# noah-aviel-dove/signals

Measured on AMD Instinct MI355X. Metric: rendered Msamples/s (48 kHz, 256-sample blocks), higher is better.
Workload: dtype f64; 1 GPU; C2: 1024-voice Fixed->Sine->LowPass->Gain->SumBus(stereo) per GPU, 48 kHz, 256-frame blocks, 4096 blocks per batch (f32 storage, f64 phase/recurrence); engine schedule = fused voice chain + bus: sig_fused_voice_bus (Sine->LowPass->Gain->SumBus in ONE launch, its voice tiles added in fixed order by the same kernel; no per-voice sample touches HBM); voices_per_gpu=1024, block_frames=256, start_position=0, parallelism=voices sharded 1024/GPU x1; single process, no collective, rccl_ranks=0

## Files before the change

### signals_amd/csrc/fused_voice.hip

```cpp
#include <cstdlib>

#include "sig_fused_launch.h"

sig_fused::Tuning& sig_fused::tuning() {
    static Tuning t = [] {
        auto env = [](const char* name, int dflt) { const char* e = getenv(name); return e ? atoi(e) : dflt; };
        Tuning u;
        u.vpt = env("SIG_FUSED_VPT", 0); u.span = env("SIG_FUSED_SPAN", 0);
        u.steady = env("SIG_FUSED_STEADY", -1); u.scan = env("SIG_FUSED_SCAN", -1);
        if (u.steady == 2) { u.steady = 1; u.tile_sum_kernel = 1; }
        if (u.steady == 3) { u.steady = 1; u.mix_f32 = 1; }
        return u;
    }();
    return t;
}

namespace {

enum Sink { SINK_VOICES, SINK_MIX, SINK_BUS };
struct FusedCall {
    int osc_kind, filt_type; int32_t rate; int64_t position;
    int32_t block_frames, nblocks, context, voices;
    const double* hertz; int32_t hertz_stride; const double* phase; int32_t phase_stride;
    const double* cutoff; int32_t cutoff_stride; const double* gain; int32_t gain_stride;
    float* out; int64_t out_ld; int32_t* status; void* stream;
    Sink sink = SINK_VOICES;
    bool rows = false;
    int32_t cutoff_rows = 1, gain_rows = 1;
    int pair_op = 0, kind2 = 0;
    const double* hertz2 = nullptr; int32_t hertz2_stride = 0; const double* phase2 = nullptr; int32_t phase2_stride = 0;
    const double* mix = nullptr; int32_t mix_stride = 0;
    int32_t hertz_rows = 1, phase_rows = 1; const double* hertz_hist = nullptr; const double* phase_hist = nullptr;
    bool devpos = false; const int64_t* position_dev = nullptr;
    const float* matrix = nullptr;
    const double* bus_gains = nullptr; int64_t bus_gains_ld = 0; int32_t bus_channels = 0; double* workspace = nullptr;
    double* consts = nullptr; int32_t consts_ready = 0; int force_walk = 0;
};

bool stride_ok(int32_t s) { return (s | 1) == 1; }

bool call_ok(const FusedCall& c)
{
    const bool bus = c.sink == SINK_BUS;
    if (c.filt_type != SIG_FILT_LOWPASS && c.filt_type != SIG_FILT_HIGHPASS) return false;
    if (!(c.rate > 0 && (c.devpos ? c.position_dev != nullptr : c.position >= 0))) return false;
    if (!(c.block_frames >= 0 && c.nblocks >= 0 && c.context >= 0 && c.voices >= 0)) return false;
    if (!(c.hertz && c.cutoff && c.out && c.out_ld >= (bus ? c.bus_channels : c.voices))) return false;
    if (!(stride_ok(c.hertz_stride) && stride_ok(c.phase_stride) && stride_ok(c.cutoff_stride) && stride_ok(c.gain_stride))) return false;
    if (!((c.cutoff_rows == 1 || c.cutoff_rows == c.nblocks) && (c.gain_rows == 1 || c.gain_rows == c.nblocks))) return false;
    if (c.pair_op != 0 && !((c.pair_op == 1 || c.pair_op == 2) && c.kind2 >= SIG_OSC_SINE && c.kind2 <= SIG_OSC_TRIANGLE && c.hertz2 &&
                            stride_ok(c.hertz2_stride) && stride_ok(c.phase2_stride) && stride_ok(c.mix_stride) && (c.pair_op == 2 || c.mix)))
        return false;
    if ((c.hertz_hist || c.phase_hist) && c.block_frames < c.context) return false;
    if (!((c.hertz_rows == 1 || (c.hertz_rows == c.nblocks && c.hertz_hist)) &&
          (c.phase_rows == 1 || (c.phase_rows == c.nblocks && c.phase_hist)) && (!c.phase_hist || c.phase))) return false;
    if (c.sink == SINK_MIX && !(c.matrix && c.voices % 64 == 0)) return false;
    if (bus && !(c.workspace && (c.bus_gains ? c.bus_gains_ld >= c.voices : c.bus_channels == 1))) return false;
    return true;
}

int run_call(const FusedCall& c)
{
    SIG_CHECK_ARG(call_ok(c));
    if (c.block_frames == 0 || c.nblocks == 0 || c.voices == 0) return 0;
    const bool bus = c.sink == SINK_BUS;
    FusedArgs a{c.filt_type, (double)c.rate, c.devpos ? 0 : c.position, c.block_frames, c.nblocks, c.context, c.voices,
                c.hertz, c.hertz_stride, c.phase, c.phase_stride, c.cutoff, c.cutoff_stride, c.gain, c.gain_stride,
                bus ? nullptr : c.out, bus ? 0 : c.out_ld, 0, c.status, c.devpos ? c.position_dev : nullptr};
    a.mix = c.matrix;
    a.consts_ext = c.consts; a.consts_ready = c.consts_ready; a.force_walk = c.force_walk;
    a.cutoff_rows = c.cutoff_rows; a.gain_rows = c.gain_rows;
    a.hertz_rows = c.hertz_rows; a.phase_rows = c.phase_rows; a.hertz_hist = c.hertz_hist; a.phase_hist = c.phase_hist;
    a.pair_op = c.pair_op; a.kind2 = c.kind2; a.hertz2 = c.hertz2; a.hs2 = c.hertz2_stride; a.phase2 = c.phase2; a.ps2 = c.phase2_stride;
    a.mixrow = c.mix; a.ms = c.mix_stride;
    const BusArgs busargs = bus ? BusArgs{c.bus_gains, c.bus_gains_ld, c.workspace, (int64_t)c.block_frames * c.nblocks}
                                : BusArgs{nullptr, 0, nullptr, 0};
    hipStream_t s = static_cast<hipStream_t>(c.stream);
    if (c.rows) {
        SIG_CHECK_ARG(!bus || c.bus_channels == 1 || c.bus_channels == 2);
        return dispatch_rows(bus ? c.bus_channels : 0, c.osc_kind, a, busargs, c.out, c.out_ld, s);
    }
    switch (c.sink) {
        case SINK_BUS: return dispatch_bus(c.gain != nullptr, c.osc_kind, c.bus_channels, a, busargs, c.out, c.out_ld, s);
        case SINK_MIX: return dispatch_mix(c.gain != nullptr, c.osc_kind, a, s);
        default: return dispatch_chain(c.gain != nullptr, c.osc_kind, a, s);
    }
}

void set_rows(FusedCall& c, int32_t cutoff_rows, int32_t gain_rows) { c.rows = true; c.cutoff_rows = cutoff_rows; c.gain_rows = gain_rows; }

void set_bus(FusedCall& c, const double* bus_gains, int64_t bus_gains_ld, int32_t bus_channels, double* workspace)
{
    c.sink = SINK_BUS; c.bus_gains = bus_gains; c.bus_gains_ld = bus_gains_ld; c.bus_channels = bus_channels; c.workspace = workspace;
}
// ... 107 lines not shown
                                      int32_t block_frames, int32_t nblocks, int32_t context, int32_t voices,
                                      const double* hertz, int32_t hertz_stride, int32_t hertz_rows, const double* hertz_hist,
                                      const double* phase, int32_t phase_stride, int32_t phase_rows, const double* phase_hist,
                                      const double* cutoff, int32_t cutoff_stride, int32_t cutoff_rows,
                                      const double* gain, int32_t gain_stride, int32_t gain_rows,
                                      const double* bus_gains, int64_t bus_gains_ld, int32_t bus_channels,
                                      double* workspace, float* out, int64_t out_ld, int32_t* status, void* stream)
{
    FusedCall c{osc_kind, filt_type, rate, position, block_frames, nblocks, context, voices, hertz, hertz_stride, phase, phase_stride,
                cutoff, cutoff_stride, gain, gain_stride, out, out_ld, status, stream};
    set_rows(c, cutoff_rows, gain_rows);
    set_fm(c, hertz_rows, hertz_hist, phase_rows, phase_hist);
    set_bus(c, bus_gains, bus_gains_ld, bus_channels, workspace);
    return run_call(c);
}

extern "C" int sig_fused_osc_biquad_devpos(int osc_kind, int filt_type, int32_t rate, const int64_t* position_dev,
                                           int32_t block_frames, int32_t nblocks, int32_t context, int32_t voices,
                                           const double* hertz, int32_t hertz_stride, const double* phase, int32_t phase_stride,
                                           const double* cutoff, int32_t cutoff_stride,
                                           const double* gain, int32_t gain_stride,
                                           float* out, int64_t out_ld, int32_t* status, void* stream)
{
    FusedCall c{osc_kind, filt_type, rate, 0, block_frames, nblocks, context, voices, hertz, hertz_stride, phase, phase_stride,
                cutoff, cutoff_stride, gain, gain_stride, out, out_ld, status, stream};
    c.devpos = true; c.position_dev = position_dev;
    return run_call(c);
}

namespace {
__global__ void advance_kernel(int64_t* p, int64_t delta) { *p += delta; }
}

extern "C" int sig_advance_position(int64_t* position_dev, int64_t delta, void* stream)
{
    SIG_CHECK_ARG(position_dev != nullptr);
    advance_kernel<<<1, 1, 0, static_cast<hipStream_t>(stream)>>>(position_dev, delta);
    return sig_launch_status();
}

extern "C" int sig_fused_osc_biquad_mix(int osc_kind, int filt_type, int32_t rate, int64_t position,
                                        int32_t block_frames, int32_t nblocks, int32_t context, int32_t voices,
                                        const double* hertz, int32_t hertz_stride, const double* phase, int32_t phase_stride,
                                        const double* cutoff, int32_t cutoff_stride,
                                        const double* gain, int32_t gain_stride,
                                        const float* matrix, float* out, int64_t out_ld, int32_t* status, void* stream)
{
    FusedCall c{osc_kind, filt_type, rate, position, block_frames, nblocks, context, voices, hertz, hertz_stride, phase, phase_stride,
                cutoff, cutoff_stride, gain, gain_stride, out, out_ld, status, stream};
    c.sink = SINK_MIX; c.matrix = matrix;
    return run_call(c);
}

extern "C" int sig_fused_geometry(int32_t voices, int32_t block_frames, int32_t nblocks, int32_t context,
                                  int32_t* voices_per_lane, int32_t* blocks_per_lane)
{
    SIG_CHECK_ARG(voices >= 0 && block_frames >= 0 && nblocks >= 0 && context >= 0 && voices_per_lane && blocks_per_lane);
    FusedArgs a{};
    a.N = block_frames; a.K = nblocks; a.ctx = context; a.voices = voices;
    int vpt = 1, span = 1;
    pick_geometry(a, 4, vpt, span);
    *voices_per_lane = vpt;
    *blocks_per_lane = span;
    return 0;
}

extern "C" int sig_fused_voice_bus_plan(int osc_kind, int64_t position, int32_t voices, int32_t block_frames, int32_t nblocks,
                                       int32_t context, int32_t* voices_per_lane, int32_t* blocks_per_lane,
                                       int32_t* closed_form)
{
    SIG_CHECK_ARG(voices >= 0 && block_frames >= 0 && nblocks >= 0 && context >= 0 && position >= 0);
    SIG_CHECK_ARG(voices_per_lane && blocks_per_lane && closed_form);
    FusedArgs a{};
    a.position = position; a.N = block_frames; a.K = nblocks; a.ctx = context; a.voices = voices;
    const BusPlan p = plan_voice_bus(a, osc_kind);
    *voices_per_lane = p.vpt;
    *blocks_per_lane = p.span;
    *closed_form = p.steady;
    return 0;
}

extern "C" int sig_fused_set_tuning(int32_t voices_per_lane, int32_t blocks_per_lane, int32_t closed_form, int32_t scan)
{
    SIG_CHECK_ARG(voices_per_lane >= 0 && blocks_per_lane >= 0 && closed_form >= -1 && closed_form <= 3 && scan >= -1);
    Tuning& t = tuning();
    t.vpt = voices_per_lane; t.span = blocks_per_lane; t.scan = scan;
    t.steady = (closed_form == 2 || closed_form == 3) ? 1 : closed_form;
    t.tile_sum_kernel = (closed_form == 2) ? 1 : 0;
    t.mix_f32 = (closed_form == 3) ? 1 : 0;
    return 0;
}

extern "C" int64_t sig_fused_voice_bus_workspace(int32_t voices, int64_t rows, int32_t bus_channels)
{
    return (steady_consts_offset(voices, rows, bus_channels) + (int64_t)kSteadyConsts * voices) * (int64_t)sizeof(double);
}

extern "C" int sig_fused_voice_bus(int osc_kind, int filt_type, int32_t rate, int64_t position,
                                   int32_t block_frames, int32_t nblocks, int32_t context, int32_t voices,
                                   const double* hertz, int32_t hertz_stride, const double* phase, int32_t phase_stride,
                                   const double* cutoff, int32_t cutoff_stride,
                                   const double* gain, int32_t gain_stride,
                                   const double* bus_gains, int64_t bus_gains_ld, int32_t bus_channels,
                                   double* workspace, float* out, int64_t out_ld, int32_t* status, void* stream)
{
    FusedCall c{osc_kind, filt_type, rate, position, block_frames, nblocks, context, voices, hertz, hertz_stride, phase, phase_stride,
                cutoff, cutoff_stride, gain, gain_stride, out, out_ld, status, stream};
    set_bus(c, bus_gains, bus_gains_ld, bus_channels, workspace);
    return run_call(c);
}

extern "C" int sig_fused_voice_bus_walk(int osc_kind, int filt_type, int32_t rate, int64_t position,
                                        int32_t block_frames, int32_t nblocks, int32_t context, int32_t voices,
                                        const double* hertz, int32_t hertz_stride, const double* phase, int32_t phase_stride,
                                        const double* cutoff, int32_t cutoff_stride,
                                        const double* gain, int32_t gain_stride,
                                        const double* bus_gains, int64_t bus_gains_ld, int32_t bus_channels,
                                        double* workspace, float* out, int64_t out_ld, int32_t* status, void* stream)
{
    FusedCall c{osc_kind, filt_type, rate, position, block_frames, nblocks, context, voices, hertz, hertz_stride, phase, phase_stride,
                cutoff, cutoff_stride, gain, gain_stride, out, out_ld, status, stream};
    set_bus(c, bus_gains, bus_gains_ld, bus_channels, workspace);
    c.force_walk = 1;
    return run_call(c);
}

extern "C" int64_t sig_fused_voice_consts_size(int32_t voices)
{
    return (int64_t)kSteadyConsts * voices * (int64_t)sizeof(double);
}

extern "C" int sig_fused_voice_bus_prepared(int osc_kind, int filt_type, int32_t rate, int64_t position,
                                            int32_t block_frames, int32_t nblocks, int32_t context, int32_t voices,
                                            const double* hertz, int32_t hertz_stride, const double* phase, int32_t phase_stride,
                                            const double* cutoff, int32_t cutoff_stride,
                                            const double* gain, int32_t gain_stride,
                                            const double* bus_gains, int64_t bus_gains_ld, int32_t bus_channels,
                                            double* workspace, float* out, int64_t out_ld, int32_t* status, void* stream,
                                            double* consts, int32_t consts_ready)
{
    SIG_CHECK_ARG(consts != nullptr);
    FusedCall c{osc_kind, filt_type, rate, position, block_frames, nblocks, context, voices, hertz, hertz_stride, phase, phase_stride,
                cutoff, cutoff_stride, gain, gain_stride, out, out_ld, status, stream};
    set_bus(c, bus_gains, bus_gains_ld, bus_channels, workspace);
    c.consts = consts; c.consts_ready = consts_ready;
    return run_call(c);
}

extern "C" int sig_fused_voice_bus_bound(const sig_fused_voice_bus_call* b, int64_t position, float* out, int32_t consts_ready,
                                         int32_t walk, void* stream)
{
    SIG_CHECK_ARG(b != nullptr && (walk || b->consts != nullptr));
    FusedCall c{b->osc_kind, b->filt_type, b->rate, position, b->block_frames, b->nblocks, b->context, b->voices, b->hertz, b->hertz_stride,
                b->phase, b->phase_stride, b->cutoff, b->cutoff_stride, b->gain, b->gain_stride, out, b->out_ld, b->status, stream};
    set_bus(c, b->bus_gains, b->bus_gains_ld, b->bus_channels, b->workspace);
    if (walk) c.force_walk = 1;
    else { c.consts = b->consts; c.consts_ready = consts_ready; }
    return run_call(c);
}
```

### signals_amd/csrc/sig_fused_launch.h

```cpp
#pragma once
#include <type_traits>

#include "sig_fused_scan.h"
#include "sig_fused_steady.h"
#include "sig_fused_walk.h"

namespace {

constexpr int64_t kWavesWanted = 2048;

int64_t waves_of(const FusedArgs& a, int v, int s) { return sig_span_waves(sig_voice_tiles(a.voices, v), a.K, s); }

void pick_geometry(const FusedArgs& a, int max_vpt, int& vpt, int& span) {
    const int env_vpt = tuning().vpt, env_span = tuning().span;
    const int max_span = (a.N >= a.ctx) ? 8 : 1;
    vpt = max_vpt; span = max_span;
    while (span > 1 && waves_of(a, vpt, span) < kWavesWanted) span >>= 1;
    while (vpt > 1 && waves_of(a, vpt, 1) < kWavesWanted / 2) vpt >>= 1;
    if (env_vpt == 1 || env_vpt == 2 || env_vpt == 4) vpt = (env_vpt <= max_vpt) ? env_vpt : max_vpt;
    if (env_span >= 1) span = (env_span <= max_span) ? env_span : max_span;
}

struct BusPlan { int vpt, span, steady; };

BusPlan plan_voice_bus(const FusedArgs& a, int kind) {
    BusPlan p{4, 1, 0};
    pick_geometry(a, 4, p.vpt, p.span);
    if (kind == SIG_OSC_SINE && !a.force_walk && (a.N >= a.ctx || a.position >= a.ctx)) {
        p.steady = tuning().steady < 0 ? 1 : tuning().steady;
        if (p.steady) {
            const int env_vpt = tuning().vpt;
            if (env_vpt == 8 || (env_vpt == 0 && p.vpt == 4 && waves_of(a, 8, p.span) >= kWavesWanted / 2)) p.vpt = 8;
            if (env_vpt == 16 || (SIG_STEADY_AUTO16 && env_vpt == 0 && p.vpt == 8 && a.voices >= SIG_WAVE * 16)) {
                int span = p.span;
                while (span > 1 && waves_of(a, 16, span) < kWavesWanted / 2) span >>= 1;
                if (env_vpt == 16 || waves_of(a, 16, span) >= kWavesWanted / 2) {
                    p.vpt = 16;
                    if (tuning().span == 0) p.span = span;
                }
            }
        }
    }
    return p;
}

template <int KIND, int C>
int launch_rows(FusedArgs a, BusArgs bus, float* out, int64_t out_ld, hipStream_t stream)
{
    if constexpr (KIND == SIG_OSC_SINE && C > 0) {
        const bool gain_only = a.gain && a.gain_rows > 1 && a.cutoff_rows == 1;
        if ((gain_only || a.cutoff_rows > 1) && !a.hertz_hist && !a.phase_hist && a.pair_op == 0) {
            BusPlan plan = plan_voice_bus(a, KIND);
            if (plan.steady) {
                if (plan.vpt > 8) plan.vpt = 8;
                if (!gain_only && tuning().vpt == 0) plan.vpt = (plan.vpt >= 8) ? 8 : (plan.vpt > 2 ? 2 : plan.vpt);
                a.span = plan.span;
                a.steady = 1;
                const int err = gain_only ? launch_steady<false, C, true>(a, bus, plan.vpt, out, out_ld, stream)
                                          : launch_steady<false, C, true, true>(a, bus, plan.vpt, out, out_ld, stream);
                if (err || bus.out) return err;
                const int tiles_s = sig_voice_tiles(a.voices, plan.vpt);
                return sig_bus::launch_partials<C>(bus.partials, tiles_s, bus.rows, out, out_ld, stream);
            }
        }
    }
    auto ok = [&](int vpt) {
        return C > 0 || ((a.voices % vpt == 0) && (a.out_ld % vpt == 0) && (reinterpret_cast<uintptr_t>(a.out) % (vpt * 4) == 0));
    };
    int max_vpt = 4;
    while (max_vpt > 1 && !ok(max_vpt)) max_vpt >>= 1;
    int vpt;
    pick_geometry(a, max_vpt, vpt, a.span);
    const int tiles = sig_voice_tiles(a.voices, vpt);
    if (C > 0 && sig_bus::tiles_sum_in_workgroup(tiles) && tuning().tile_sum_kernel == 0) { bus.out = out; bus.out_ld = out_ld; }
    const int err = launch_walk<KIND, false, C, true>(a, bus, vpt, stream);
    if (err || C == 0 || bus.out) return err;
    return sig_bus::launch_partials<(C > 0 ? C : 1)>(bus.partials, tiles, bus.rows, out, out_ld, stream);
}

template <int KIND, bool GAIN, int C>
int launch_voice_bus(FusedArgs a, BusArgs bus, float* out, int64_t out_ld, hipStream_t stream)
{
    const BusPlan plan = plan_voice_bus(a, KIND);
    const int vpt = plan.vpt;
    a.span = plan.span;
    a.steady = plan.steady;
    bool done = false;
    if constexpr (KIND == SIG_OSC_SINE) {
        if (a.steady) {
            const int e2 = launch_steady<GAIN, C, false>(a, bus, vpt, out, out_ld, stream);
            if (e2 || bus.out) return e2;
            done = true;
        }
    }
    if (!done) {
        const int tiles_w = sig_voice_tiles(a.voices, vpt);
        if (sig_bus::tiles_sum_in_workgroup(tiles_w) && tuning().tile_sum_kernel == 0) { bus.out = out; bus.out_ld = out_ld; }
        const int err = launch_walk<KIND, GAIN, C>(a, bus, vpt, stream);
        if (err || bus.out) return err;
    }
    const int tiles = sig_voice_tiles(a.voices, vpt);
    return sig_bus::launch_partials<C>(bus.partials, tiles, bus.rows, out, out_ld, stream);
}
// ... 113 lines not shown
```

### signals_amd/csrc/sig_fused_steady.h

```cpp
#pragma once
#include <type_traits>

#include "sig_biquad.h"
#include "sig_bus_tile.h"
#include "sig_osc.h"
#include "sig_steady.h"

namespace {

using namespace sig_fused;
using sig_bus::kPairs;
using sig_bus::kTileStride;

enum { SC_NA1, SC_NA2, SC_SCALE, SC_K2C, SC_ST, SC_CT, SC_HRE, SC_HIM, SC_ND, SC_T, SC_T0 = SC_T + 4, kSteadyConsts = SC_T0 + 4 };

__device__ __forceinline__ bool steady_wave(const FusedArgs& a, int v0, int vpt, int64_t p0, int nb) {
    const double q_first = (double)p0 / a.rate, q_last = (double)(p0 + (int64_t)nb * a.N - 1) / a.rate;
    bool ok = true;
    for (int i = 0; i < vpt; ++i) {
        const int v = (v0 + i < a.voices) ? v0 + i : ((v0 < a.voices) ? v0 : 0);
        ok &= steady_voice_ok(a.hertz[(int64_t)v * a.hs], a.phase ? a.phase[(int64_t)v * a.ps] : 0.0, a.rate,
                              a.steady_consts[(int64_t)SC_ST * a.voices + v], q_first, q_last);
    }
    return __all(ok);
}

template <bool GAIN>
__global__ __launch_bounds__(256) void steady_prep_kernel(FusedArgs a, double* __restrict__ consts)
{
    const int v = blockIdx.x * blockDim.x + threadIdx.x;
    if (v >= a.voices) return;
    const SteadyVoice c = steady_constants<GAIN>(a, v);
    if (!c.ok && a.status) atomicOr(a.status, SIG_STATUS_BAD_CUTOFF);
    auto put = [&](int k, double x) { consts[(int64_t)k * a.voices + v] = x; };
    put(SC_NA1, c.na1); put(SC_NA2, c.na2); put(SC_SCALE, c.scale);
    put(SC_K2C, c.k2c); put(SC_ST, c.st); put(SC_CT, c.ct);
    put(SC_HRE, c.hre); put(SC_HIM, c.him); put(SC_ND, c.nd);
    put(SC_T + 0, c.T.a); put(SC_T + 1, c.T.b); put(SC_T + 2, c.T.c); put(SC_T + 3, c.T.d);
    put(SC_T0 + 0, c.T0.a); put(SC_T0 + 1, c.T0.b); put(SC_T0 + 2, c.T0.c); put(SC_T0 + 3, c.T0.d);
}

template <int VPT, int C>
__device__ __forceinline__ void steady_fallback_span(const FusedArgs& a, const BusArgs& bus, double* tile, int lane, int vt,
                                                  int64_t b_first, int nb, int v0)
{
    const int vc = (v0 < a.voices) ? v0 : 0;
    const double* sc = a.steady_consts;
    const double s2 = (a.type == SIG_FILT_LOWPASS) ? 2.0 : -2.0;
    sig_bus::PipelinedTile<C> stage(tile, lane, bus.partials + (int64_t)vt * bus.rows * C, b_first * a.N);
    for (int i = 0; i < VPT; ++i)
        if (v0 + i < a.voices && a.status && sc[(int64_t)SC_NA1 * a.voices + v0 + i] != sc[(int64_t)SC_NA1 * a.voices + v0 + i])
            atomicOr(a.status, SIG_STATUS_BAD_CUTOFF);
#pragma unroll 1
    for (int bi = 0; bi < nb; ++bi) {
        const int64_t p_b = a.position + (b_first + bi) * a.N;
        const int c = (int)((p_b < (int64_t)a.ctx) ? p_b : (int64_t)a.ctx);
        double z0[VPT], z1[VPT];
#pragma unroll
        for (int i = 0; i < VPT; ++i) z0[i] = z1[i] = 0.0;
#pragma unroll 1
        for (int r = -c; r < a.N; ++r) {
            const double q = (double)(p_b + r) / a.rate;
            double acc[C];
#pragma unroll
            for (int ch = 0; ch < C; ++ch) acc[ch] = 0.0;
#pragma unroll
            for (int i = 0; i < VPT; ++i) {
                const bool live = v0 + i < a.voices;
                const int v = live ? v0 + i : vc;
                const double t = q * a.hertz[(int64_t)v * a.hs] + (a.phase ? a.phase[(int64_t)v * a.ps] : 0.0);
                const double x = (double)sig_osc::osc_sine_f32(t);
                double na1 = sc[(int64_t)SC_NA1 * a.voices + v], na2 = sc[(int64_t)SC_NA2 * a.voices + v];
                double scale = live ? sc[(int64_t)SC_SCALE * a.voices + v] : 0.0;
                if (a.cutoff_rows > 1) {
                    Biquad qd;
                    design_butter2(a.type, a.cutoff[(b_first + bi) * (int64_t)(a.cs ? a.voices : 1) + (int64_t)v * a.cs], a.rate, qd);
                    na1 = -qd.a1; na2 = -qd.a2;
                    scale = live ? qd.b0 : 0.0;
                    if (a.gain && a.gain_rows == 1) scale *= a.gain[(int64_t)v * a.gs];
                }
                const double y = x + z0[i];
                z0[i] = fma(na1, y, fma(s2, x, z1[i]));
                z1[i] = fma(na2, y, x);
                if (a.gain_rows > 1) scale *= a.gain[(b_first + bi) * (int64_t)(a.gs ? a.voices : 1) + (int64_t)v * a.gs];
#pragma unroll
                for (int ch = 0; ch < C; ++ch) acc[ch] = fma(bus.pan ? bus.pan[ch * bus.pan_ld + v] * scale : scale, y, acc[ch]);
            }
            if (r >= 0) {
#pragma unroll
                for (int ch = 0; ch < C; ++ch) stage.slot[ch * kTileStride] = acc[ch];
                stage.advance();
            }
        }
    }
    if (stage.staged) stage.now();
}

template <int VPT> struct SteadyVariants {
    static constexpr int count = (VPT >= 8) ? 7 : (VPT == 4) ? 4 : (VPT == 2) ? 3 : 2;
    static constexpr int at(int k) {
        constexpr int v8[7] = {8, 6, 4, 3, 2, 1, 0}, v4[4] = {4, 2, 1, 0}, v2[3] = {2, 1, 0}, v1[2] = {1, 0};
        return (VPT >= 8) ? v8[k] : (VPT == 4) ? v4[k] : (VPT == 2) ? v2[k] : v1[k];
    }
};

#ifndef SIG_STEADY_OCC8
#define SIG_STEADY_OCC8 1
#endif
#ifndef SIG_STEADY_AUTO16
#define SIG_STEADY_AUTO16 0
#endif
#ifndef SIG_STEADY_OCC16
#define SIG_STEADY_OCC16 1
#endif
template <int VPT> struct SteadyOcc { static constexpr int waves = (VPT == 16) ? SIG_STEADY_OCC16 : (VPT == 8) ? SIG_STEADY_OCC8 : 2; };

template <int VPT, int C, bool GROWS, bool CROWS = false>
__device__ __forceinline__ void steady_bus_wave(const FusedArgs& a, const BusArgs& bus, double* tile, int lane, int wave, double* osc_store = nullptr)
{
    constexpr bool OSC_LDS = CROWS && VPT >= 8;
    constexpr int R = kPairs / C;
    constexpr int LC = SteadyVariants<VPT>::at(0);
    static_assert(R % 2 == 0, "the two-term recurrence rotates two registers per voice: row groups are even");
    const int64_t item = (int64_t)blockIdx.x * 4 + wave;
    const int vt = (int)(item % a.voice_tiles);
    const int64_t b_first = (item / a.voice_tiles) * a.span;
    if (b_first >= a.K) return;
    const int nb = (int)((a.K - b_first < (int64_t)a.span) ? a.K - b_first : (int64_t)a.span);
    const int v0 = (vt * SIG_WAVE + lane) * VPT;
    const int vc = (v0 < a.voices) ? v0 : 0;
    const int64_t p0 = a.position + b_first * a.N;
    if (!steady_wave(a, v0, VPT, p0, nb)) {
        steady_fallback_span<VPT, C>(a, bus, tile, lane, vt, b_first, nb, v0);
        return;
    }
    const double* sc = a.steady_consts;

    double na1[LC], na2[LC], k2c[VPT], ya[VPT], yb[VPT], wt[C][VPT];
    int nd_total[VPT];
    const double q_first = (double)p0 / a.rate;
#pragma unroll
    for (int i = 0; i < VPT; ++i) {
        const bool live = v0 + i < a.voices;
        const int v = live ? v0 + i : vc;
        auto cst = [&](int k) { return sc[(int64_t)k * a.voices + v]; };
        const double na1_i = cst(SC_NA1);
        if (i < LC) { na1[i < LC ? i : 0] = na1_i; na2[i < LC ? i : 0] = cst(SC_NA2); }
        k2c[i] = cst(SC_K2C);
        if (live && na1_i != na1_i && a.status) atomicOr(a.status, SIG_STATUS_BAD_CUTOFF);
        const double scale = cst(SC_SCALE);
#pragma unroll
        for (int ch = 0; ch < C; ++ch)
            wt[ch][i] = live ? (bus.pan ? bus.pan[ch * bus.pan_ld + v] * scale : scale) : 0.0;
        const double hz = a.hertz[(int64_t)v * a.hs], ph = a.phase ? a.phase[(int64_t)v * a.ps] : 0.0;
        const double t_first = q_first * hz + ph;
        const double f0 = t_first - rint(t_first);
        const double ur = sin2pi(f0 + 0.25), ui = sin2pi(f0);
        const double hre = cst(SC_HRE), him = cst(SC_HIM);
        const double wr = fma(hre, ur, -(him * ui)), wi = fma(hre, ui, him * ur);
        yb[i] = wi;
        ya[i] = fma(wi, cst(SC_CT), -(wr * cst(SC_ST)));
        const double nd = cst(SC_ND);
        nd_total[i] = (live && nd < (double)kNeverDrops) ? (int)nd : (live ? kNeverDrops : 0);
    }
#pragma unroll
    for (int d = 1; d < SIG_WAVE; d <<= 1) {
        int other[VPT];
#pragma unroll
        for (int i = 0; i < VPT; ++i) other[i] = __shfl_xor(nd_total[i], d, SIG_WAVE);
#pragma unroll
        for (int i = 0; i < VPT; ++i) nd_total[i] = (other[i] > nd_total[i]) ? other[i] : nd_total[i];
    }
#pragma unroll
    for (int i = 0; i < VPT; ++i) nd_total[i] = __builtin_amdgcn_readfirstlane(nd_total[i]);

    double* dstp = bus.partials + (int64_t)vt * bus.rows * C;
    sig_bus::PipelinedTile<C> stage(tile, lane, dstp, b_first * a.N);

    if constexpr (LC < VPT) {
        const int c_min = (b_first == 0 && a.position < (int64_t)a.ctx) ? (int)a.position : a.ctx;
        bool capped = true;
#pragma unroll
        for (int i = LC; i < VPT; ++i) capped &= nd_total[i] <= c_min;
        if (!capped) {
            steady_fallback_span<VPT, C>(a, bus, tile, lane, vt, b_first, nb, v0);
            return;
        }
    }
    [[maybe_unused]] OscPart osc[(CROWS && !OSC_LDS) ? VPT : 1];
    auto osc_slot = [&](int field, int i) -> double& { return osc_store[((size_t)field * VPT + i) * SIG_WAVE + lane]; };
    if constexpr (CROWS) {
#pragma unroll
        for (int i = 0; i < VPT; ++i) {
            const int v = (v0 + i < a.voices) ? v0 + i : vc;
            const OscPart made = steady_osc_part(a.type, a.hertz[(int64_t)v * a.hs], a.rate, a.ctx);
            if constexpr (OSC_LDS) {
                osc_slot(0, i) = made.ct; osc_slot(1, i) = made.st; osc_slot(2, i) = made.beta; osc_slot(3, i) = made.enr; osc_slot(4, i) = made.eni;
            } else {
                osc[i] = made;
            }
        }
    }
    double z0h[LC], z1h[LC];
    auto row = [&](double* sums, int sums_stride, auto m_tag, auto odd_tag) {
        constexpr int M = decltype(m_tag)::value;
        constexpr bool ODD = decltype(odd_tag)::value;
        double y[VPT];
#pragma unroll
        for (int i = 0; i < VPT; ++i) {
            const double ys = ODD ? ya[i] : yb[i];
            if (ODD) yb[i] = fma(k2c[i], ya[i], -yb[i]);
            else ya[i] = fma(k2c[i], yb[i], -ya[i]);
            if (i < M) {
                const int j = i < LC ? i : 0;
                y[i] = ys + z0h[j];
                const double yh = z0h[j];
                z0h[j] = fma(na1[j], yh, z1h[j]);
                z1h[j] = na2[j] * yh;
            } else {
                y[i] = ys;
            }
        }
#pragma unroll
        for (int ch = 0; ch < C; ++ch) {
            double acc = 0.0;
#pragma unroll
            for (int i = 0; i < VPT; ++i) acc = fma(wt[ch][i], y[i], acc);
            sums[ch * sums_stride] = acc;
        }
    };
    sig_bus::FoldedGroup<C> folded(tile, lane, dstp);
    double pend[4];
    int64_t pend_row = 0;
    bool have = false;
    auto rows2 = [&](double* sums, auto m_tag) {
        constexpr int M = decltype(m_tag)::value;
        double y0[VPT], y1[VPT];
#pragma unroll
        for (int i = 0; i < VPT; ++i) {
            y0[i] = yb[i];
            ya[i] = fma(k2c[i], yb[i], -ya[i]);
            y1[i] = ya[i];
            yb[i] = fma(k2c[i], ya[i], -yb[i]);
            if (i < M) {
                const int j = i < LC ? i : 0;
                const double h0 = z0h[j];
                y0[i] += h0;
                const double h1 = fma(na1[j], h0, z1h[j]);
                y1[i] += h1;
                z0h[j] = fma(na1[j], h1, na2[j] * h0);
                z1h[j] = na2[j] * h1;
            }
        }
        double acc0[C], acc1[C];
#pragma unroll
        for (int ch = 0; ch < C; ++ch) { acc0[ch] = 0.0; acc1[ch] = 0.0; }
#pragma unroll
        for (int i = 0; i < VPT; ++i) {
#pragma unroll
            for (int ch = 0; ch < C; ++ch) {
                acc0[ch] = fma(wt[ch][i], y0[i], acc0[ch]);
                acc1[ch] = fma(wt[ch][i], y1[i], acc1[ch]);
            }
        }
#pragma unroll
        for (int ch = 0; ch < C; ++ch) { sums[ch] = acc0[ch]; sums[C + ch] = acc1[ch]; }
    };
    auto group = [&](auto m_tag) {
        double acc[kPairs];
#pragma unroll
        for (int k = 0; k < R; k += 2) {
            rows2(acc + k * C, m_tag);
#pragma unroll
            for (int q = 0; q < kPairs / 4; ++q)
                if (4 * q + 3 < (k + 2) * C && 4 * q + 3 >= k * C)
                    folded.fold4(q, acc[4 * q], acc[4 * q + 1], acc[4 * q + 2], acc[4 * q + 3]);
            if (k + 2 == R / 2 && have) folded.finish(pend, pend_row, R);
        }
        folded.issue(pend);
        pend_row = stage.first; stage.first += R; have = true;
    };
    using Variants = SteadyVariants<VPT>;

    for (int bi = 0; bi < nb; ++bi) {
        if constexpr (GROWS && !CROWS) {
#pragma unroll
            for (int i = 0; i < VPT; ++i) {
                const bool live = v0 + i < a.voices;
                const int v = live ? v0 + i : vc;
                const double scale = sc[(int64_t)SC_SCALE * a.voices + v] * a.gain[(b_first + bi) * (int64_t)(a.gs ? a.voices : 1) + (int64_t)v * a.gs];
#pragma unroll
                for (int ch = 0; ch < C; ++ch) wt[ch][i] = live ? (bus.pan ? bus.pan[ch * bus.pan_ld + v] * scale : scale) : 0.0;
            }
        }
        const bool first = (b_first + bi == 0);
        const int tk = first ? SC_T0 : SC_T;
        const int c = first ? (int)((a.position < (int64_t)a.ctx) ? a.position : (int64_t)a.ctx) : a.ctx;
        if constexpr (CROWS) {
            const int64_t blk = b_first + bi;
            const double q_b = (double)(p0 + (int64_t)bi * a.N) / a.rate;
            double cut_i[VPT], gain_i[VPT];
#pragma unroll
            for (int i = 0; i < VPT; ++i) {
                const int v = (v0 + i < a.voices) ? v0 + i : vc;
                cut_i[i] = a.cutoff[(a.cutoff_rows > 1 ? blk * (int64_t)(a.cs ? a.voices : 1) : 0) + (int64_t)v * a.cs];
                gain_i[i] = a.gain ? a.gain[(a.gain_rows > 1 ? blk * (int64_t)(a.gs ? a.voices : 1) : 0) + (int64_t)v * a.gs] : 1.0;
            }
#pragma unroll
            for (int i = 0; i < VPT; ++i) {
                const bool live = v0 + i < a.voices;
                const int v = live ? v0 + i : vc;
                const double cutoff = cut_i[i], gain = gain_i[i];
                const double hz_v = a.hertz[(int64_t)v * a.hs], ph_v = a.phase ? a.phase[(int64_t)v * a.ps] : 0.0;
                OscPart op;
                if constexpr (OSC_LDS) op = OscPart{osc_slot(0, i), osc_slot(1, i), osc_slot(2, i), osc_slot(3, i), osc_slot(4, i)};
                else op = osc[i];
                if (__builtin_expect(c != a.ctx, 0)) op = steady_osc_part(a.type, hz_v, a.rate, c);
                const double ct_i = op.ct, st_i = op.st;
                const BlockVoice cv = steady_block_constants(a.type, a.rate, cutoff, gain, op, c);
                if (i < LC) { na1[i < LC ? i : 0] = cv.na1; na2[i < LC ? i : 0] = cv.na2; }
                if (live && !cv.ok && a.status) atomicOr(a.status, SIG_STATUS_BAD_CUTOFF);
#pragma unroll
                for (int ch = 0; ch < C; ++ch) wt[ch][i] = live ? (bus.pan ? bus.pan[ch * bus.pan_ld + v] * cv.scale : cv.scale) : 0.0;
                const double t_first = q_b * hz_v + ph_v;
                const double f0 = t_first - rint(t_first);
                const double ur = sin2pi(f0 + 0.25), ui = sin2pi(f0);
                const double wr = fma(cv.hre, ur, -(cv.him * ui)), wi = fma(cv.hre, ui, cv.him * ur);
                yb[i] = wi;
                ya[i] = fma(wi, ct_i, -(wr * st_i));
                if (i < LC) {
                    const double dss = fma(k2c[i], yb[i], -ya[i]) - yb[i];
                    z0h[i < LC ? i : 0] = fma(cv.T.a, yb[i], cv.T.b * dss);
                    z1h[i < LC ? i : 0] = fma(cv.T.c, yb[i], cv.T.d * dss);
                }
                nd_total[i] = (live && cv.nd < (double)kNeverDrops) ? (int)cv.nd : (live ? kNeverDrops : 0);
            }
#pragma unroll
            for (int d = 1; d < SIG_WAVE; d <<= 1) {
                int other[VPT];
#pragma unroll
                for (int i = 0; i < VPT; ++i) other[i] = __shfl_xor(nd_total[i], d, SIG_WAVE);
#pragma unroll
                for (int i = 0; i < VPT; ++i) nd_total[i] = (other[i] > nd_total[i]) ? other[i] : nd_total[i];
            }
#pragma unroll
            for (int i = 0; i < VPT; ++i) nd_total[i] = __builtin_amdgcn_readfirstlane(nd_total[i]);
        }
        int drop_at[LC];
#pragma unroll
        for (int i = 0; i < LC; ++i) {
            drop_at[i] = (nd_total[i] > c) ? nd_total[i] - c : 0;
            if (drop_at[i] > 0) {
                const int v = (v0 + i < a.voices) ? v0 + i : vc;
                const double dss = fma(k2c[i], yb[i], -ya[i]) - yb[i];
                if constexpr (!CROWS) {
                    const double* t = sc + (int64_t)tk * a.voices + v;
                    z0h[i] = fma(t[0], yb[i], t[a.voices] * dss);
                    z1h[i] = fma(t[2 * (int64_t)a.voices], yb[i], t[3 * (int64_t)a.voices] * dss);
                }
            } else {
                z0h[i] = 0.0; z1h[i] = 0.0;
            }
        }
        int done = 0;
        auto single = [&]() {
            row(stage.slot, kTileStride, std::integral_constant<int, LC>{}, std::false_type{});
#pragma unroll
            for (int i = 0; i < VPT; ++i) { const double t = ya[i]; ya[i] = yb[i]; yb[i] = t; }
            ++done;
            stage.advance();
        };
        while (stage.staged != 0 && done < a.N) single();
        const int last_group_row = done + ((a.N - done) / R) * R;
        auto phase = [&](auto k_tag) {
            constexpr int K = decltype(k_tag)::value;
            constexpr int M = Variants::at(K);
            constexpr int lower = (K + 1 < Variants::count) ? Variants::at(K + 1) : 0;
            int until = 0;
#pragma unroll
            for (int i = lower; i < LC; ++i) until = (i < M && drop_at[i] > until) ? drop_at[i] : until;
            if (M == 0) until = a.N;
            until = (until < last_group_row) ? until : last_group_row;
            while (done < until) {
                group(std::integral_constant<int, M>{});
                done += R;
            }
        };
#define SIG_PHASE(K) if constexpr (K < Variants::count) phase(std::integral_constant<int, K>{});
        SIG_PHASE(0) SIG_PHASE(1) SIG_PHASE(2) SIG_PHASE(3) SIG_PHASE(4) SIG_PHASE(5) SIG_PHASE(6) SIG_PHASE(7) SIG_PHASE(8)
#undef SIG_PHASE
        if (done < a.N) {
            if (have) { folded.finish(pend, pend_row, R); have = false; }
#pragma unroll
            for (int i = 0; i < LC; ++i)
                if (drop_at[i] <= done) { z0h[i] = 0.0; z1h[i] = 0.0; }
            while (done < a.N) single();
        }
    }
    if (have) folded.finish(pend, pend_row, R);
    if (stage.staged) stage.now();
}

template <int VPT, int C, bool GROWS = false, bool CROWS = false>
__global__ __launch_bounds__(256) __attribute__((amdgpu_waves_per_eu(CROWS ? 1 : SteadyOcc<VPT>::waves, 8)))
void fused_steady_bus_kernel(FusedArgs a, BusArgs bus)
{
    __shared__ double lds[4][kPairs * kTileStride];
    constexpr bool kOscInLds = CROWS && VPT >= 8;
    __shared__ double osc_lds[kOscInLds ? 4 * 5 * VPT * SIG_WAVE : 1];
    const int lane = threadIdx.x & 63;
    const int wave = __builtin_amdgcn_readfirstlane(threadIdx.x >> 6);
    steady_bus_wave<VPT, C, GROWS, CROWS>(a, bus, lds[wave], lane, wave,
                                          kOscInLds ? osc_lds + (size_t)wave * 5 * VPT * SIG_WAVE : nullptr);
    if (bus.out) sig_bus::sum_tiles_in_workgroup<C>(bus.partials, a.voice_tiles, bus.rows, a.span, a.K, a.N, bus.out, bus.out_ld, lane, wave);
}

int64_t steady_consts_offset(int voices, int64_t rows, int bus_channels) {
    return (int64_t)sig_voice_tiles(voices, 1) * rows * bus_channels;
}

template <bool GAIN, int C, bool GROWS, bool CROWS = false>
int launch_steady(FusedArgs& a, BusArgs& bus, int vpt, float* out, int64_t out_ld, hipStream_t stream)
{
    double* consts = a.consts_ext ? a.consts_ext : bus.partials + steady_consts_offset(a.voices, bus.rows, C);
    a.steady_consts = consts;
    if (!(a.consts_ext && a.consts_ready))
        steady_prep_kernel<GAIN><<<(a.voices + 255) / 256, 256, 0, stream>>>(a, consts);

    a.voice_tiles = sig_voice_tiles(a.voices, vpt);
    unsigned nwg;
    if (!sig_workgroups(sig_span_waves(a.voice_tiles, a.K, a.span), nwg)) return (int)hipErrorInvalidValue;
    if (sig_bus::tiles_sum_in_workgroup(a.voice_tiles) && tuning().tile_sum_kernel == 0) { bus.out = out; bus.out_ld = out_ld; }
    switch (vpt) {
        case 1: fused_steady_bus_kernel<1, C, GROWS, CROWS><<<nwg, 256, 0, stream>>>(a, bus); break;
        case 2: fused_steady_bus_kernel<2, C, GROWS, CROWS><<<nwg, 256, 0, stream>>>(a, bus); break;
        case 8: fused_steady_bus_kernel<8, C, GROWS, CROWS><<<nwg, 256, 0, stream>>>(a, bus); break;
        case 16: if constexpr (!CROWS) { fused_steady_bus_kernel<16, C, GROWS><<<nwg, 256, 0, stream>>>(a, bus); break; }
        default: fused_steady_bus_kernel<4, C, GROWS, CROWS><<<nwg, 256, 0, stream>>>(a, bus); break;
    }
    return sig_launch_status();
}

}
```

### signals_amd/csrc/sig_steady.h

```cpp
#pragma once
#include "sig_biquad.h"
#include "sig_osc.h"

namespace sig_fused {

using sig_biquad::Biquad;
using sig_biquad::design_butter2;

struct FusedArgs {
    int type; double rate; int64_t position; int N, K, ctx, voices;
    const double* hertz; int hs; const double* phase; int ps;
    const double* cutoff; int cs; const double* gain; int gs;
    float* out; int64_t out_ld; int voice_tiles; int* status;
    const int64_t* pos_dev = nullptr;
    const float* mix = nullptr;
    int span = 1;
    int steady = 0;
    const double* steady_consts = nullptr;
    double* consts_ext = nullptr;
    int consts_ready = 0;
    int force_walk = 0;
    int cutoff_rows = 1, gain_rows = 1;
    int hertz_rows = 1, phase_rows = 1;
    const double* hertz_hist = nullptr; const double* phase_hist = nullptr;
    int pair_op = 0, kind2 = 0;
    const double* hertz2 = nullptr; int hs2 = 0; const double* phase2 = nullptr; int ps2 = 0; const double* mixrow = nullptr; int ms = 0;
};

struct BusArgs {
    const double* pan; int64_t pan_ld; double* partials; int64_t rows;
    float* out = nullptr; int64_t out_ld = 0;
};

struct Tuning { int vpt = 0, span = 0, steady = -1, scan = -1, tile_sum_kernel = 0, mix_f32 = 0; };
Tuning& tuning();
int part_b_rows(int C, int kind, const FusedArgs& a, const BusArgs& bus, float* out, int64_t out_ld, hipStream_t s);
int part_b_bus(int gain, int kind, int C, const FusedArgs& a, const BusArgs& bus, float* out, int64_t out_ld, hipStream_t s);
int part_b_mix(int gain, int kind, const FusedArgs& a, hipStream_t s);
int part_b_chain(int gain, int kind, const FusedArgs& a, hipStream_t s);

__device__ __forceinline__ double sin2pi(double f) {
    const double u = fma(f, 2.0, sig_osc::kRoundMagic);
    const double k = u - sig_osc::kRoundMagic;
    const double rq = fma(k, -0.5, f);
    const double y = sig_osc::sin_poly(fma(rq, sig_osc::kTwoPiHi, rq * sig_osc::kTwoPiLo));
    return __hiloint2double(__double2hiint(y) ^ (int)(((unsigned)__double2loint(u) & 1u) << 31), __double2loint(y));
}

struct M2 { double a, b, c, d; };
__device__ __forceinline__ M2 m2_mul(const M2& x, const M2& y) {
    return {fma(x.a, y.a, x.b * y.c), fma(x.a, y.b, x.b * y.d), fma(x.c, y.a, x.d * y.c), fma(x.c, y.b, x.d * y.d)};
}

constexpr double kHomogeneousTol = 1e-9;

__device__ __forceinline__ bool steady_voice_ok(double hz, double ph, double rate, double st, double q_first, double q_last) {
    const double t_first = q_first * hz + ph, t_last = q_last * hz + ph;
    const double d = hz / rate;
    const double dr = d - rint(d);
    return fabs(t_first) < sig_osc::kSineFastMaxT && fabs(t_last) < sig_osc::kSineFastMaxT && fabs(dr) <= 0.25 &&
           fabs(st) >= 1e-3;
}

struct SteadyVoice { bool ok; double na1, na2, scale, k2c, st, ct, hre, him, nd; M2 T, T0; };

template <bool GAIN>
__device__ __forceinline__ SteadyVoice steady_constants_of(const FusedArgs& a, int v, double cutoff, double gain, int c_first)
{
    using sig_biquad::Cx; using sig_biquad::cx_mul; using sig_biquad::cx_div;
    SteadyVoice r;
    Biquad q;
    r.ok = design_butter2(a.type, cutoff, a.rate, q);
    const double s2 = (a.type == SIG_FILT_LOWPASS) ? 2.0 : -2.0;
    const double a1 = q.a1, a2 = q.a2;
    const double d = a.hertz[(int64_t)v * a.hs] / a.rate;
    const double dr = d - rint(d);
    const double st = sin2pi(dr), ct = sin2pi(dr + 0.25), sh = sin2pi(0.5 * dr);
    const Cx z = {ct, -st};
    const Cx z2 = cx_mul(z, z);
    const Cx H = cx_div({1.0 + s2 * z.re + z2.re, s2 * z.im + z2.im}, {1.0 + a1 * z.re + a2 * z2.re, a1 * z.im + a2 * z2.im});
    const Cx P = {H.re - 1.0, H.im};
    const Cx Pe = cx_mul(P, {ct, st});
    const Cx Q = {Pe.re - s2 + a1 * H.re, Pe.im + a1 * H.im};
    const double alpha = 2.0 * sh * sh / st, beta = 1.0 / st;
    auto make_T = [&](int c) {
        const double cf = (double)c * dr;
        const Cx E = cx_div({sin2pi(cf + 0.25), -sin2pi(cf)}, H);
        const Cx PE = cx_mul(P, E), QE = cx_mul(Q, E);
        const M2 Mss = {fma(PE.im, alpha, PE.re), PE.im * beta, fma(QE.im, alpha, QE.re), QE.im * beta};
        M2 Ac = {1.0, 0.0, 0.0, 1.0}, Ap = {-a1, 1.0, -a2, 0.0};
        for (int e = c; e > 0; e >>= 1) {
            if (e & 1) Ac = m2_mul(Ac, Ap);
            Ap = m2_mul(Ap, Ap);
        }
        const M2 t = m2_mul(Ac, Mss);
        return M2{-t.a, -t.b, -t.c, -t.d};
    };
    r.T = make_T(a.ctx);
    r.T0 = (c_first == a.ctx) ? r.T : make_T(c_first);
    r.nd = __builtin_inf();
    {
        const double d2 = a2 - 0.25 * a1 * a1;
        if (r.ok && d2 > 0.0 && a2 > 0.0 && a2 < 1.0) {
            const double dd = sqrt(d2), f2 = 1.0 + 0.25 * a1 * a1 + d2;
            const double kappa = (f2 + sqrt(fmax(f2 * f2 - 4.0 * d2, 0.0))) / (2.0 * dd);
            const double amp = q.b0 * kappa * sqrt(P.re * P.re + P.im * P.im + Q.re * Q.re + Q.im * Q.im);
            const double rows = (amp > kHomogeneousTol) ? log(kHomogeneousTol / amp) / (0.5 * log(a2)) : 0.0;
            if (rows == rows) r.nd = ceil(rows) + 1.0;
        }
    }
    r.na1 = -a1; r.na2 = -a2;
    r.scale = GAIN ? q.b0 * gain : q.b0;
    r.k2c = 2.0 * ct; r.st = st; r.ct = ct; r.hre = H.re; r.him = H.im;
    return r;
}

template <bool GAIN>
__device__ __forceinline__ SteadyVoice steady_constants(const FusedArgs& a, int v)
{
    const int c0 = (int)((a.position < (int64_t)a.ctx) ? a.position : (int64_t)a.ctx);
    return steady_constants_of<GAIN>(a, v, a.cutoff[(int64_t)v * a.cs], GAIN ? a.gain[(int64_t)v * a.gs] : 1.0, c0);
}

struct OscPart { double ct, st, beta, enr, eni; };
struct BlockVoice { bool ok; double na1, na2, scale, hre, him; M2 T; double nd; };

__device__ __forceinline__ OscPart steady_osc_part(int type, double hertz, double rate, int c)
{
    using sig_biquad::Cx; using sig_biquad::cx_mul; using sig_biquad::cx_div;
    const double d = hertz / rate, dr = d - rint(d);
    OscPart o;
    o.st = sin2pi(dr); o.ct = sin2pi(dr + 0.25);
    o.beta = 1.0 / o.st;
    const double s2 = (type == SIG_FILT_LOWPASS) ? 2.0 : -2.0;
    const Cx z = {o.ct, -o.st}, z2 = cx_mul(z, z);
    const Cx N = {1.0 + s2 * z.re + z2.re, s2 * z.im + z2.im};
    const double cf = (double)c * dr;
    const Cx E = cx_div({sin2pi(cf + 0.25), -sin2pi(cf)}, N);
    o.enr = E.re; o.eni = E.im;
    return o;
}

__device__ __forceinline__ BlockVoice steady_block_constants(int type, double rate, double cutoff, double gain, const OscPart& o, int c)
{
// ... 79 lines not shown
```

Before: 2.569 million Msamples/s.

## Step steady-state oscillators every D rows via cosine-sum recurrence in fused bus kernel

Adds a path in the steady voice-bus kernel where each sine oscillator advances D rows at a time using a 2cos(D·w) Chebyshev recurrence. The intermediate rows' bus contributions are reconstructed from precomputed per-voice cosine weights and shared homogeneous filter terms, which cuts the per-row dependent FMA chain per voice. Extra per-voice constants (cosines, sin(D·w), transient coefficients) are computed in the prep kernel, and the path is used only when every voice in the wave has a well-conditioned sin(D·w). It also raises the cap on a forced span and adds a tuning switch to fall back to row-by-row stepping. Costs are more registers and constant loads, plus some numerical risk when sin(D·w) is small.

```diff
diff --git a/signals_amd/csrc/fused_voice.hip b/signals_amd/csrc/fused_voice.hip
--- a/signals_amd/csrc/fused_voice.hip
+++ b/signals_amd/csrc/fused_voice.hip
@@ -10,6 +10,7 @@
         u.steady = env("SIG_FUSED_STEADY", -1); u.scan = env("SIG_FUSED_SCAN", -1);
         if (u.steady == 2) { u.steady = 1; u.tile_sum_kernel = 1; }
         if (u.steady == 3) { u.steady = 1; u.mix_f32 = 1; }
+        if (u.steady == 4) { u.steady = 1; u.row_by_row = 1; }
         return u;
     }();
     return t;
@@ -283,12 +284,13 @@
 
 extern "C" int sig_fused_set_tuning(int32_t voices_per_lane, int32_t blocks_per_lane, int32_t closed_form, int32_t scan)
 {
-    SIG_CHECK_ARG(voices_per_lane >= 0 && blocks_per_lane >= 0 && closed_form >= -1 && closed_form <= 3 && scan >= -1);
+    SIG_CHECK_ARG(voices_per_lane >= 0 && blocks_per_lane >= 0 && closed_form >= -1 && closed_form <= 4 && scan >= -1);
     Tuning& t = tuning();
     t.vpt = voices_per_lane; t.span = blocks_per_lane; t.scan = scan;
-    t.steady = (closed_form == 2 || closed_form == 3) ? 1 : closed_form;
+    t.steady = (closed_form >= 2 && closed_form <= 4) ? 1 : closed_form;
     t.tile_sum_kernel = (closed_form == 2) ? 1 : 0;
     t.mix_f32 = (closed_form == 3) ? 1 : 0;
+    t.row_by_row = (closed_form == 4) ? 1 : 0;
     return 0;
 }
 
diff --git a/signals_amd/csrc/sig_fused_launch.h b/signals_amd/csrc/sig_fused_launch.h
--- a/signals_amd/csrc/sig_fused_launch.h
+++ b/signals_amd/csrc/sig_fused_launch.h
@@ -18,7 +18,8 @@
     while (span > 1 && waves_of(a, vpt, span) < kWavesWanted) span >>= 1;
     while (vpt > 1 && waves_of(a, vpt, 1) < kWavesWanted / 2) vpt >>= 1;
     if (env_vpt == 1 || env_vpt == 2 || env_vpt == 4) vpt = (env_vpt <= max_vpt) ? env_vpt : max_vpt;
-    if (env_span >= 1) span = (env_span <= max_span) ? env_span : max_span;
+    const int max_forced = (a.N >= a.ctx) ? 64 : 1;
+    if (env_span >= 1) span = (env_span <= max_forced) ? env_span : max_forced;
 }
 
 struct BusPlan { int vpt, span, steady; };
diff --git a/signals_amd/csrc/sig_fused_steady.h b/signals_amd/csrc/sig_fused_steady.h
--- a/signals_amd/csrc/sig_fused_steady.h
+++ b/signals_amd/csrc/sig_fused_steady.h
@@ -12,7 +12,8 @@
 using sig_bus::kPairs;
 using sig_bus::kTileStride;
 
-enum { SC_NA1, SC_NA2, SC_SCALE, SC_K2C, SC_ST, SC_CT, SC_HRE, SC_HIM, SC_ND, SC_T, SC_T0 = SC_T + 4, kSteadyConsts = SC_T0 + 4 };
+enum { SC_NA1, SC_NA2, SC_SCALE, SC_K2C, SC_ST, SC_CT, SC_HRE, SC_HIM, SC_ND, SC_T, SC_T0 = SC_T + 4,
+       SC_C2 = SC_T0 + 4, SC_SD = SC_C2 + 3, SC_DSA, SC_DSB, kSteadyConsts };
 
 __device__ __forceinline__ bool steady_wave(const FusedArgs& a, int v0, int vpt, int64_t p0, int nb) {
     const double q_first = (double)p0 / a.rate, q_last = (double)(p0 + (int64_t)nb * a.N - 1) / a.rate;
@@ -38,6 +39,9 @@
     put(SC_HRE, c.hre); put(SC_HIM, c.him); put(SC_ND, c.nd);
     put(SC_T + 0, c.T.a); put(SC_T + 1, c.T.b); put(SC_T + 2, c.T.c); put(SC_T + 3, c.T.d);
     put(SC_T0 + 0, c.T0.a); put(SC_T0 + 1, c.T0.b); put(SC_T0 + 2, c.T0.c); put(SC_T0 + 3, c.T0.d);
+    const SteadyCosines k = steady_cosines(a.hertz[(int64_t)v * a.hs], a.rate, SIG_STEADY_D);
+    put(SC_C2 + 0, k.c2[0]); put(SC_C2 + 1, k.c2[1]); put(SC_C2 + 2, k.c2[2]);
+    put(SC_SD, k.sd); put(SC_DSA, k.dsa); put(SC_DSB, k.dsb);
 }
 
 template <int VPT, int C>
@@ -115,13 +119,35 @@
 #endif
 template <int VPT> struct SteadyOcc { static constexpr int waves = (VPT == 16) ? SIG_STEADY_OCC16 : (VPT == 8) ? SIG_STEADY_OCC8 : 2; };
 
-template <int VPT, int C, bool GROWS, bool CROWS = false>
+template <int VPT, int C> struct SteadyRows {
+    static constexpr int R = kPairs / C;
+    static constexpr int D = (VPT <= 8 && R % SIG_STEADY_D == 0 && (R / SIG_STEADY_D) % 2 == 0) ? SIG_STEADY_D : 1;
+};
+
+template <int VPT, int C>
+__device__ __forceinline__ bool steady_cosine_wave(const FusedArgs& a, int lane, int wave)
+{
+    if (SteadyRows<VPT, C>::D == 1 || !a.cosine_rows || a.N % (kPairs / C) != 0) return false;
+    const int64_t item = (int64_t)blockIdx.x * 4 + wave;
+    const int v0 = ((int)(item % a.voice_tiles) * SIG_WAVE + lane) * VPT;
+    bool ok = true;
+#pragma unroll
+    for (int i = 0; i < VPT; ++i) {
+        const int v = (v0 + i < a.voices) ? v0 + i : ((v0 < a.voices) ? v0 : 0);
+        ok &= fabs(a.steady_consts[(int64_t)SC_SD * a.voices + v]) >= 1e-3;
+    }
+    return __all(ok);
+}
+
+template <int VPT, int C, bool GROWS, bool CROWS = false, int D = 1>
 __device__ __forceinline__ void steady_bus_wave(const FusedArgs& a, const BusArgs& bus, double* tile, int lane, int wave, double* osc_store = nullptr)
 {
     constexpr bool OSC_LDS = CROWS && VPT >= 8;
     constexpr int R = kPairs / C;
     constexpr int LC = SteadyVariants<VPT>::at(0);
     static_assert(R % 2 == 0, "the two-term recurrence rotates two registers per voice: row groups are even");
+    static_assert(D == 1 || (!GROWS && !CROWS && VPT <= 8 && R % D == 0 && (R / D) % 2 == 0), "cosine-sum rows: see above");
+    constexpr int DD = D;
     const int64_t item = (int64_t)blockIdx.x * 4 + wave;
     const int vt = (int)(item % a.voice_tiles);
     const int64_t b_first = (item / a.voice_tiles) * a.span;
@@ -280,8 +306,111 @@
         folded.issue(pend);
         pend_row = stage.first; stage.first += R; have = true;
     };
+    [[maybe_unused]] double kd[D > 1 ? VPT : 1], wj[D > 1 ? D - 1 : 1][C][D > 1 ? VPT : 1];
+    [[maybe_unused]] double hs[D > 1 ? D : 1][C];
+    [[maybe_unused]] auto centre = [&](double* sums, auto m_tag, auto odd_tag) __attribute__((always_inline)) {
+        constexpr int M = decltype(m_tag)::value;
+        constexpr bool ODD = decltype(odd_tag)::value;
+        double yc[VPT];
+#pragma unroll
+        for (int i = 0; i < VPT; ++i) yc[i] = ODD ? ya[i] : yb[i];
+        double hh[D][M > 0 ? M : 1];
+#pragma unroll
+        for (int i = 0; i < M; ++i) {
+            const int j = i < LC ? i : 0;
+            hh[0][i] = z0h[j];
+            hh[1][i] = fma(na1[j], hh[0][i], z1h[j]);
+#pragma unroll
+            for (int r = 2; r < D; ++r) hh[r][i] = fma(na1[j], hh[r - 1][i], na2[j] * hh[r - 2][i]);
+            z0h[j] = fma(na1[j], hh[D - 1][i], na2[j] * hh[D - 2][i]);
+            z1h[j] = na2[j] * hh[D - 1][i];
+        }
+        double acc[D][C], nh[D][C];
+#pragma unroll
+        for (int ch = 0; ch < C; ++ch) {
+            acc[0][ch] = 0.0;
+#pragma unroll
+            for (int r = 1; r < D; ++r) acc[r][ch] = -hs[D - r][ch];
+        }
+#pragma unroll
+        for (int i = 0; i < VPT; ++i) {
+            const double y0 = (i < M) ? yc[i] + hh[0][i < M ? i : 0] : yc[i];
+#pragma unroll
+            for (int ch = 0; ch < C; ++ch) {
+                acc[0][ch] = fma(wt[ch][i], y0, acc[0][ch]);
+#pragma unroll
+                for (int r = 1; r < D; ++r) acc[r][ch] = fma(wj[r - 1][ch][i], yc[i], acc[r][ch]);
+            }
+        }
+#pragma unroll
+        for (int ch = 0; ch < C; ++ch) {
+#pragma unroll
+            for (int r = 1; r < D; ++r) {
+                nh[r][ch] = acc[r][ch];
+#pragma unroll
+                for (int i = 0; i < M; ++i) acc[r][ch] = fma(wt[ch][i], hh[r][i], acc[r][ch]);
+            }
+        }
+#pragma unroll
+        for (int r = 0; r < D; ++r) {
+#pragma unroll
+            for (int ch = 0; ch < C; ++ch) {
+                sums[r * C + ch] = acc[r][ch];
+                if (r > 0) hs[r][ch] = nh[r][ch];
+            }
+        }
+#pragma unroll
+        for (int i = 0; i < VPT; ++i) {
+            if (ODD) yb[i] = fma(kd[i], ya[i], -yb[i]);
+            else ya[i] = fma(kd[i], yb[i], -ya[i]);
+        }
+    };
+    auto fold_rows = [&](const double* acc, int k0, int k1) __attribute__((always_inline)) {
+#pragma unroll
+        for (int q = 0; q < kPairs / 4; ++q)
+            if (4 * q + 3 < k1 * C && 4 * q + 3 >= k0 * C)
+                folded.fold4(q, acc[4 * q], acc[4 * q + 1], acc[4 * q + 2], acc[4 * q + 3]);
+        if (k1 == R / 2 && have) folded.finish(pend, pend_row, R);
+    };
+    [[maybe_unused]] auto group_d = [&](auto m_tag) __attribute__((always_inline)) {
+        double acc[kPairs];
+#pragma unroll
+        for (int k = 0; k < R; k += 2 * D) {
+            centre(acc + k * C, m_tag, std::false_type{});
+            fold_rows(acc, k, k + D);
+            centre(acc + (k + D) * C, m_tag, std::true_type{});
+            fold_rows(acc, k + D, k + 2 * D);
+        }
+        folded.issue(pend);
+        pend_row = stage.first; stage.first += R; have = true;
+    };
     using Variants = SteadyVariants<VPT>;
 
+    if constexpr (D > 1) {
+#pragma unroll
+        for (int r = 0; r < D; ++r)
+#pragma unroll
+            for (int ch = 0; ch < C; ++ch) hs[r][ch] = 0.0;
+#pragma unroll
+        for (int i = 0; i < VPT; ++i) {
+            const int v = (v0 + i < a.voices) ? v0 + i : vc;
+            double ym[D + 1];
+            ym[0] = yb[i]; ym[1] = ya[i];
+#pragma unroll
+            for (int j = 2; j <= D; ++j) ym[j] = fma(k2c[i], ym[j - 1], -ym[j - 2]);
+            ya[i] = ym[D];
+            kd[i] = sc[(int64_t)(SC_C2 + D - 2) * a.voices + v];
+#pragma unroll
+            for (int j = 1; j < D; ++j) {
+                const double cj = (j == 1) ? k2c[i] : sc[(int64_t)(SC_C2 + (j > 1 ? j - 2 : 0)) * a.voices + v];
+#pragma unroll
+                for (int ch = 0; ch < C; ++ch) {
+                    wj[j - 1][ch][i] = wt[ch][i] * cj;
+                    hs[j][ch] = fma(wt[ch][i], ym[D - j], hs[j][ch]);
+                }
+            }
+        }
+    }
     for (int bi = 0; bi < nb; ++bi) {
         if constexpr (GROWS && !CROWS) {
 #pragma unroll
@@ -352,7 +481,14 @@
             drop_at[i] = (nd_total[i] > c) ? nd_total[i] - c : 0;
             if (drop_at[i] > 0) {
                 const int v = (v0 + i < a.voices) ? v0 + i : vc;
-                const double dss = fma(k2c[i], yb[i], -ya[i]) - yb[i];
+                double dss;
+                if constexpr (DD > 1) {
+                    dss = fma(sc[(int64_t)SC_DSA * a.voices + v], yb[i], sc[(int64_t)SC_DSB * a.voices + v] * ya[i]);
+                    na1[i] = sc[(int64_t)SC_NA1 * a.voices + v];
+                    na2[i] = sc[(int64_t)SC_NA2 * a.voices + v];
+                } else {
+                    dss = fma(k2c[i], yb[i], -ya[i]) - yb[i];
+                }
                 if constexpr (!CROWS) {
                     const double* t = sc + (int64_t)tk * a.voices + v;
                     z0h[i] = fma(t[0], yb[i], t[a.voices] * dss);
@@ -360,6 +496,7 @@
                 }
             } else {
                 z0h[i] = 0.0; z1h[i] = 0.0;
+                if constexpr (DD > 1) { na1[i] = 0.0; na2[i] = 0.0; }
             }
         }
         int done = 0;
@@ -370,7 +507,7 @@
             ++done;
             stage.advance();
         };
-        while (stage.staged != 0 && done < a.N) single();
+        if constexpr (DD == 1) while (stage.staged != 0 && done < a.N) single();
         const int last_group_row = done + ((a.N - done) / R) * R;
         auto phase = [&](auto k_tag) {
             constexpr int K = decltype(k_tag)::value;
@@ -382,14 +519,15 @@
             if (M == 0) until = a.N;
             until = (until < last_group_row) ? until : last_group_row;
             while (done < until) {
-                group(std::integral_constant<int, M>{});
+                if constexpr (DD > 1) group_d(std::integral_constant<int, M>{});
+                else group(std::integral_constant<int, M>{});
                 done += R;
             }
         };
 #define SIG_PHASE(K) if constexpr (K < Variants::count) phase(std::integral_constant<int, K>{});
         SIG_PHASE(0) SIG_PHASE(1) SIG_PHASE(2) SIG_PHASE(3) SIG_PHASE(4) SIG_PHASE(5) SIG_PHASE(6) SIG_PHASE(7) SIG_PHASE(8)
 #undef SIG_PHASE
-        if (done < a.N) {
+        if constexpr (DD == 1) if (done < a.N) {
             if (have) { folded.finish(pend, pend_row, R); have = false; }
 #pragma unroll
             for (int i = 0; i < LC; ++i)
@@ -410,8 +548,15 @@
     __shared__ double osc_lds[kOscInLds ? 4 * 5 * VPT * SIG_WAVE : 1];
     const int lane = threadIdx.x & 63;
     const int wave = __builtin_amdgcn_readfirstlane(threadIdx.x >> 6);
-    steady_bus_wave<VPT, C, GROWS, CROWS>(a, bus, lds[wave], lane, wave,
-                                          kOscInLds ? osc_lds + (size_t)wave * 5 * VPT * SIG_WAVE : nullptr);
+    bool cosine = false;
+    if constexpr (!GROWS && !CROWS && SteadyRows<VPT, C>::D > 1) {
+        if (steady_cosine_wave<VPT, C>(a, lane, wave)) {
+            steady_bus_wave<VPT, C, false, false, SteadyRows<VPT, C>::D>(a, bus, lds[wave], lane, wave);
+            cosine = true;
+        }
+    }
+    if (!cosine)
+        steady_bus_wave<VPT, C, GROWS, CROWS>(a, bus, lds[wave], lane, wave, kOscInLds ? osc_lds + (size_t)wave * 5 * VPT * SIG_WAVE : nullptr);
     if (bus.out) sig_bus::sum_tiles_in_workgroup<C>(bus.partials, a.voice_tiles, bus.rows, a.span, a.K, a.N, bus.out, bus.out_ld, lane, wave);
 }
 
@@ -424,6 +569,7 @@
 {
     double* consts = a.consts_ext ? a.consts_ext : bus.partials + steady_consts_offset(a.voices, bus.rows, C);
     a.steady_consts = consts;
+    a.cosine_rows = tuning().row_by_row ? 0 : 1;
     if (!(a.consts_ext && a.consts_ready))
         steady_prep_kernel<GAIN><<<(a.voices + 255) / 256, 256, 0, stream>>>(a, consts);
 
diff --git a/signals_amd/csrc/sig_steady.h b/signals_amd/csrc/sig_steady.h
--- a/signals_amd/csrc/sig_steady.h
+++ b/signals_amd/csrc/sig_steady.h
@@ -20,6 +20,7 @@
     double* consts_ext = nullptr;
     int consts_ready = 0;
     int force_walk = 0;
+    int cosine_rows = 0;
     int cutoff_rows = 1, gain_rows = 1;
     int hertz_rows = 1, phase_rows = 1;
     const double* hertz_hist = nullptr; const double* phase_hist = nullptr;
@@ -32,7 +33,7 @@
     float* out = nullptr; int64_t out_ld = 0;
 };
 
-struct Tuning { int vpt = 0, span = 0, steady = -1, scan = -1, tile_sum_kernel = 0, mix_f32 = 0; };
+struct Tuning { int vpt = 0, span = 0, steady = -1, scan = -1, tile_sum_kernel = 0, mix_f32 = 0, row_by_row = 0; };
 Tuning& tuning();
 int part_b_rows(int C, int kind, const FusedArgs& a, const BusArgs& bus, float* out, int64_t out_ld, hipStream_t s);
 int part_b_bus(int gain, int kind, int C, const FusedArgs& a, const BusArgs& bus, float* out, int64_t out_ld, hipStream_t s);
@@ -60,6 +61,23 @@
     const double dr = d - rint(d);
     return fabs(t_first) < sig_osc::kSineFastMaxT && fabs(t_last) < sig_osc::kSineFastMaxT && fabs(dr) <= 0.25 &&
            fabs(st) >= 1e-3;
+}
+
+#ifndef SIG_STEADY_D
+#define SIG_STEADY_D 4
+#endif
+static_assert(SIG_STEADY_D == 2 || SIG_STEADY_D == 4, "cosine-sum rows: the oscillators step every 2nd or every 4th row");
+struct SteadyCosines { double c2[3], sd, dsa, dsb; };
+__device__ __forceinline__ SteadyCosines steady_cosines(double hertz, double rate, int D) {
+    const double d = hertz / rate, dr = d - rint(d);
+    SteadyCosines r;
+    for (int j = 2; j <= 4; ++j) r.c2[j - 2] = 2.0 * sin2pi((double)j * dr + 0.25);
+    const double st = sin2pi(dr), sh = sin2pi(0.5 * dr), cd = sin2pi((double)D * dr + 0.25);
+    r.sd = sin2pi((double)D * dr);
+    const double ratio = st / r.sd;
+    r.dsa = fma(ratio, cd, -2.0 * sh * sh);
+    r.dsb = -ratio;
+    return r;
 }
 
 struct SteadyVoice { bool ok; double na1, na2, scale, k2c, st, ct, hre, him, nd; M2 T, T0; };
```

Measured after the change: 2.594 million Msamples/s (median of 6 runs). Within noise of the previous version (+1.0%).
